# nextpyp/cet_pick

Measured on AMD Instinct MI355X. Metric: subtomograms/sec (MoCo-3D train) + voxels/sec (heatmap+NMS) at 1/2/4/8 GPU, higher is better.
Workload: dtype f32; 1 GPU; moco_main.py moco3d_18: 3D encoder, synthetic 512x512x128 tomogram, 32^3 subtomo crops, batch 64 per GPU, r=1024, dim=128, m=0.999, T=0.1, SGD lr 1e-3; global_batch=64, parallelism=dp1, hipgraph=True

## Files before the change

cet_pick_amd/_lib.py:

```python
import ctypes
import os

import torch

_HERE = os.path.dirname(os.path.abspath(__file__))
LIB_PATH = os.environ.get("CETPICK_HIP_LIB") or os.path.join(_HERE, "libcetpick_hip.so")

_c = ctypes
_P, _I, _F, _Z, _D, _L = _c.c_void_p, _c.c_int, _c.c_float, _c.c_size_t, _c.c_double, _c.c_long


class ConvGeom(ctypes.Structure):
    _fields_ = [(f, _I) for f in "N Di Hi Wi Ci Co kd kh kw stride pd ph pw dd dh dw".split()]


_G = _c.POINTER(ConvGeom)


class Aug2d3dRanges(ctypes.Structure):
    _fields_ = [(f, _F) for f in "flip_p angle_lo angle_hi erase_p scale_lo scale_hi ratio_lo ratio_hi".split()]


_R = _c.POINTER(Aug2d3dRanges)

# ... 127 lines not shown
    "mi_bn_bwd_apply": (_I, [_P, _P, _P, _P, _L, _I, _P, _P, _P, _D, _I, _P, _P, _P]),
    "mi_bn_bwd_apply_res": (_I, [_P, _P, _P, _P, _P, _L, _I, _P, _P, _P, _D, _P, _P, _P]),
    "mi_bn_param_grads": (_I, [_P, _I, _P, _P, _P]),
    "mi_colsum": (_I, [_P, _L, _I, _P, _P, _P, _Z, _P]),
    "mi_maxpool3d_fwd": (_I, [_P, _P, _P] + [_I] * 8 + [_P]),
    "mi_maxpool3d_bwd": (_I, [_P, _P, _P] + [_I] * 8 + [_P]),
    "mi_avgpool_fwd": (_I, [_P, _P, _I, _I, _I, _P]),
    "mi_avgpool_bwd": (_I, [_P, _P, _I, _I, _I, _P]),
    "mi_bias_add": (_I, [_P, _P, _L, _I, _P]),
    "mi_copy_pair_f32": (_I, [_P, _P, _P, _P, _L, _P]),
    "mi_relu_mask": (_I, [_P, _P, _P, _P, _L, _P]),
    "mi_l2norm_fwd": (_I, [_P, _P, _P, _I, _I, _P]),
    "mi_l2norm_bwd": (_I, [_P, _P, _P, _P, _I, _I, _P]),
    "mi_moco_logits_fwd": (_I, [_P, _P, _P, _P, _I, _I, _I, _F, _P]),
    "mi_moco_logits_norm_fwd": (_I, [_P, _P, _P, _P, _P, _P, _P, _I, _I, _I, _F, _P]),
    "mi_moco_logits_bwd": (_I, [_P, _P, _P, _P, _I, _I, _I, _F, _P]),
    "mi_rowdot_mean_fwd": (_I, [_P, _P, _P, _I, _I, _P]),
    "mi_rowdot_mean_bwd": (_I, [_P, _P, _P, _I, _I, _P]),
    "mi_column_std_mean": (_I, [_P, _P, _I, _I, _P]),
    "mi_ce_label0_fwd": (_I, [_P, _P, _P, _P, _P, _I, _I, _P, _P]),
    "mi_ce_label0_bwd": (_I, [_P, _P, _P, _P, _I, _I, _P]),
    "mi_conv3d_s2_dgrad_usable": (_I, [_I, _I, _I, _I]),
    "mi_conv3d_s2_dgrad_workspace_bytes": (_Z, [_I, _I]),
    "mi_conv3d_s2_dgrad_f32": (_I, [_P] * 7 + [_I, _I, _I, _I, _P, _Z, _P]),
    "mi_conv3d_s2_fwd_usable": (_I, [_I, _I, _I, _I]),
    "mi_conv3d_s2_fwd_workspace_bytes": (_Z, [_I, _I]),
    "mi_conv3d_s2_fwd_f32": (_I, [_P] * 5 + [_I, _I, _I, _I, _P, _Z, _P]),
    "mi_conv3d_s2_prep": (_I, [_P] * 6 + [_I, _P]),
    "mi_conv3d_s2_fwd_img_f32": (_I, [_P] * 4 + [_I] * 4 + [_P]),
    "mi_conv3d_s2_dgrad_img_f32": (_I, [_P] * 6 + [_I] * 4 + [_P]),
    "mi_ema_update": (_I, [_P, _P, _F, _L, _P]),
    "mi_sgd_step": (_I, [_P, _P, _P, _F, _F, _F, _L, _P]),
    "mi_sgd_step2": (_I, [_P, _P, _P, _P, _F, _F, _F, _L, _P]),
    "mi_scalar_accumulate": (_I, [_P, _P, _P, _P, _P, _P]),
    "mi_queue_enqueue": (_I, [_P, _P, _P, _I, _I, _I, _P]),
    "mi_kmeans_image_bytes": (_Z, [_I, _I]),
    "mi_kmeans_workspace_bytes": (_Z, [_L, _I, _I]),
    "mi_kmeans_prep": (_I, [_P, _I, _I, _P, _P]),
    "mi_kmeans_xnorm": (_I, [_P, _L, _I, _P, _P]),
    "mi_kmeans_assign": (_I, [_P, _P, _P, _L, _I, _I, _P, _P, _P, _Z, _P]),
    "mi_kmeans_update": (_I, [_P, _P, _L, _I, _I, _P, _P, _P, _P, _P, _Z, _P]),
    "mi_knn_image_bytes": (_Z, [_L, _I]),
    "mi_knn_workspace_bytes": (_Z, [_L, _L, _I, _I, _I, _I]),
    "mi_knn_search": (_I, [_P, _P, _L, _L, _I, _I, _I, _I, _I, _P, _P, _P, _Z, _P]),
    "mi_tsne_affinities": (_I, [_P, _L, _I, _F, _P, _P, _P]),
    "mi_tsne_workspace_bytes": (_Z, [_L, _I, _I]),
    "mi_tsne_gradient": (_I, [_P, _P, _P, _P, _P, _L, _I, _F, _I, _P, _P, _P, _P, _Z, _P]),
    "mi_tsne_update": (_I, [_P, _P, _P, _P, _L, _F, _F, _F, _P]),
    "mi_umap_check": (_I, [_L, _I]),
    "mi_umap_smooth_knn": (_I, [_P, _L, _I, _D, _P, _P, _P, _P]),
    "mi_umap_union": (_I, [_P, _P, _P, _P, _L, _I, _P, _I, _P, _P, _P, _P]),
    "mi_umap_rowmax": (_I, [_P, _P, _P, _P, _P, _L, _I, _D, _D, _P, _P]),
    "mi_umap_supervise": (_I, [_P, _P, _P, _P, _L, _I, _D, _D, _P, _I, _P, _P, _P]),
    "mi_umap_epoch": (_I, [_P, _P, _P, _P, _P, _P, _P, _L, _I, _I, _I, _D, _D, _c.c_uint64, _P]),
    "mi_graph_components": (_I, [_P, _P, _P, _P, _P, _L, _I, _P, _P, _P, _P]),
    "mi_spectral_degree": (_I, [_P, _P, _P, _P, _P, _P, _L, _I, _P, _P, _P]),
    "mi_spectral_spmv": (_I, [_P, _P, _P, _P, _P, _P, _L, _I, _P, _P, _P, _L, _L, _P]),
    "mi_spectral_workspace_bytes": (_Z, [_I, _L]),
    "mi_spectral_dots": (_I, [_P, _L, _I, _L, _P, _P, _P, _Z, _P]),
    "mi_spectral_orth": (_I, [_P, _L, _I, _L, _P, _P, _P, _Z, _P]),
    "mi_spectral_combine": (_I, [_P, _L, _I, _L, _P, _P, _D, _P]),
    "mi_vis_sample_colours": (_I, [_P, _L, _P, _I, _I, _P, _P]),
    "mi_vis_slice_bytes": (_I, [_P, _L, _L, _P, _D, _D, _P, _P]),
    "mi_vis_gauss_workspace_bytes": (_Z, [_L, _L, _L]),
    "mi_vis_gauss_u8": (_I, [_P, _I, _I, _I, _P, _P, _P, _Z, _P]),
    "mi_vis_paint": (_I, [_P, _P, _L, _P, _I, _I, _I, _I, _I, _I, _P, _P, _P]),
# ... 100 lines not shown
```

cet_pick_amd/csrc/conv_direct3.hip:

```cpp
#include "common.h"
#include "bf16x3.h"
#include <type_traits>
#include <algorithm>

namespace {

using namespace bf3;

constexpr int C = 64;
constexpr int PLANE = 64;
constexpr int TZ = 2;
constexpr int PZ = TZ + 2;
constexpr int NV = PZ * PLANE;
constexpr int LEAD = 16;
constexpr int ZREC = 34;
constexpr int NREC = LEAD + NV + ZREC;
constexpr int ARR = NREC * 16;
constexpr int KS = C / 16;
constexpr int PL_BYTES = 2 * ARR;
constexpr int KS_BYTES = 3 * PL_BYTES;
constexpr int LDS_BYTES = KS * KS_BYTES;
constexpr int ZBASE = (LEAD + NV) * 16;
constexpr int WBLK = 1024;
constexpr int WSTEP = 2 * 3 * WBLK;
constexpr int NTAP = 27;
constexpr int NSTEP = KS * NTAP;
constexpr int WIMG_BYTES = NSTEP * WSTEP;
constexpr int RB = 6;
static_assert(NSTEP % RB == 0, "ring slots");
static_assert(LDS_BYTES <= 160 * 1024, "patch must fit the CU's LDS");
static_assert(((LEAD + NV) & 15) == 0, "zero region must start at a record = 0 (mod 16)");

struct Direct3Params {
    const float* a;
// ... 399 lines not shown
            if (has_mask) v = (mm[r] > 0.f) ? v : 0.f;
            if (eo[r] != 0x80000000u) p.out[eo[r] / 4] = v;
        }
    }
}

constexpr int PREP_MAX = 16;
struct PrepBatch {
    const float* w[PREP_MAX];
    unsigned char* img[PREP_MAX];
    int dgrad[PREP_MAX];
    int wide[PREP_MAX];
};
__device__ void direct3s_prep_body(const float* w, unsigned char* img, int dgrad, int idx);
__device__ void direct3s256_prep_body(const float* w, unsigned char* img, int dgrad, int idx);
constexpr int PREP_BLOCKS_256 = 8 * NTAP * 2 * 8 * 64 / 256;
constexpr int PREP_BLOCKS = NTAP * KS * 2 * 64 / 256;
constexpr int PREP_BLOCKS_WIDE = 4 * NTAP * 2 * 4 * 64 / 256;
template <int CT>
__device__ void direct3_prep_body(const float* w, unsigned char* img, int dgrad, int idx) {
    constexpr int KSn = CT / 16;
    const int lane = idx & 63, cw = (idx >> 6) & 1, rest = idx >> 7, ks = rest % KSn, tap = (rest / KSn) % NTAP, cb = rest / (KSn * NTAP);
    if (cb >= CT / 64) return;
    const int nn = cb * 64 + cw * 32 + (lane & 31), k0 = ks * 16 + 8 * (lane >> 5);
    float v[8];
    if (dgrad) {
        ld8(w + ((long)(NTAP - 1 - tap) * CT + nn) * CT + k0, v);
    } else {
#pragma unroll
        for (int e = 0; e < 8; ++e) v[e] = w[((long)tap * CT + k0 + e) * CT + nn];
    }
    u32x4 o[3];
    cut8(v, o);
    unsigned char* dst = img + (long)(((cb * KSn + ks) * NTAP + tap) * 2 + cw) * (3 * WBLK) + lane * 16;
    store_planes(dst, WBLK, o);
}
__global__ __launch_bounds__(256) void direct3_prep_kernel(PrepBatch b) {
    const int fmt = b.wide[blockIdx.y], idx = blockIdx.x * 256 + threadIdx.x;
    if (fmt == 1) { if (blockIdx.x < PREP_BLOCKS_WIDE) direct3s_prep_body(b.w[blockIdx.y], b.img[blockIdx.y], b.dgrad[blockIdx.y], idx); }
    else if (fmt == 2) { if (blockIdx.x < PREP_BLOCKS_WIDE) direct3_prep_body<128>(b.w[blockIdx.y], b.img[blockIdx.y], b.dgrad[blockIdx.y], idx); }
    else if (fmt == 3) direct3s256_prep_body(b.w[blockIdx.y], b.img[blockIdx.y], b.dgrad[blockIdx.y], idx);
    else if (blockIdx.x < PREP_BLOCKS) direct3_prep_body<C>(b.w[blockIdx.y], b.img[blockIdx.y], b.dgrad[blockIdx.y], idx);
}

constexpr int WG_SPLITS = 28;
constexpr int WROW = 64;
constexpr int WHALF = (PLANE + 1) * WROW;
constexpr int WPL = 2 * WHALF;
constexpr int WOP = 3 * WPL;
constexpr int WBUF = 2 * WOP;
constexpr int WZERO = PLANE * WROW;

constexpr int WG_MAXPROB = 4;
struct Direct3WgradParams {
    const float* x[WG_MAXPROB];
    const float* dy[WG_MAXPROB];
    float* slabs[WG_MAXPROB];
    int N, D;
    unsigned bytes;
    int nprob, splits;
    int H, W;
};

constexpr int W_HB = 3 * 2 * 8 * 128;
template <bool V4, int CT, bool TILED = false>
__global__ __launch_bounds__(512, 2) void direct3_wgrad_kernel(Direct3WgradParams p) {
    __shared__ __attribute__((aligned(16))) unsigned char lds[2 * WBUF + (TILED ? 2 * W_HB : 16)];
    unsigned char* const halo = lds + 2 * WBUF;
// ... 423 lines not shown
    for (int i = 0; i < 2; ++i)
#pragma unroll
        for (int r = 0; r < 16; ++r) red[(cc * 32 + i * 16 + r) * 64 + lane] = acc[i][r];
    __syncthreads();
    const long m0 = (long)n0 * VS;
    const int col = ct * 32 + l32;
#pragma unroll
    for (int j = 0; j < 8; ++j) {
        const int idx = cc * 8 + j, i = idx >> 4, r = idx & 15;
        float t = ((red[idx * 64 + lane] + red[(32 + idx) * 64 + lane]) + red[(64 + idx) * 64 + lane]) + red[(96 + idx) * 64 + lane];
        const long o = (m0 + 32 * i + (r & 3) + 8 * (r >> 2) + 4 * h) * CT + col;
        if (p.res) t += p.res[o];
        if (p.relu) t = fmaxf(t, 0.f);
        if (p.mask) t = (p.mask[o] > 0.f) ? t : 0.f;
        p.out[o] = t;
    }
}

template <int CT>
__device__ void direct3s_prep_body_t(const float* w, unsigned char* img, int dgrad, int idx) {
    constexpr int NCB = CT / 32;
    const int lane = idx & 63, cb = (idx >> 6) % NCB, r1 = (idx >> 6) / NCB, ksx = r1 & 1, rest = r1 >> 1, tap = rest % NTAP, cc = rest / NTAP;
    if (cc >= NCB) return;
    const int nn = cb * 32 + (lane & 31), k0 = cc * 32 + ksx * 16 + 8 * (lane >> 5);
    float v[8];
    if (dgrad) {
        ld8(w + ((long)(NTAP - 1 - tap) * CT + nn) * CT + k0, v);
    } else {
#pragma unroll
        for (int e = 0; e < 8; ++e) v[e] = w[((long)tap * CT + k0 + e) * CT + nn];
    }
    u32x4 o[3];
    cut8(v, o);
    unsigned char* dst = img + (long)(((cc * NTAP + tap) * 2 + ksx) * NCB + cb) * (3 * WBLK) + lane * 16;
    store_planes(dst, WBLK, o);
}
__device__ void direct3s_prep_body(const float* w, unsigned char* img, int dgrad, int idx) { direct3s_prep_body_t<CS>(w, img, dgrad, idx); }
__device__ void direct3s256_prep_body(const float* w, unsigned char* img, int dgrad, int idx) { direct3s_prep_body_t<256>(w, img, dgrad, idx); }

}

int mi_direct3_kind(int N, int Di, int Hi, int Wi, int Ci, int Co, int kd, int kh, int kw, int stride, int pd, int ph,
                    int pw, int dd, int dh, int dw) {
    const char* off = getenv("MI_CONV_NO_DIRECT");
    if (off && atoi(off) != 0) return 0;
    if (kd != 3 || kh != 3 || kw != 3 || stride != 1 || pd != 1 || ph != 1 || pw != 1 || dd != 1 || dh != 1 || dw != 1) return 0;
    if (N < 1 || 4l * N * Di * Hi * Wi * Ci >= 0x7fff0000l) return 0;
    if (Ci == C && Co == C && Hi == 8 && Wi == 8 && Di >= TZ && Di % TZ == 0) return 1;
    if (Ci == CS && Co == CS && Di == 4 && Hi == 4 && Wi == 4) return 2;
    if (Ci == 128 && Co == 128 && Hi == 8 && Wi == 8 && Di >= TZ && Di % TZ == 0 && (long)N * Di >= 128 && (long)N * (Di / TZ) <= 0x7fffffffl) return 3;
    if (Ci == 256 && Co == 256 && Di == 4 && Hi == 4 && Wi == 4 && N >= 16) return 4;
    if (Ci == C && Co == C && (Hi > 8 || Wi > 8) && Hi >= 8 && Wi >= 8 && Di >= TZ && Di % TZ == 0) {
        const bool ragged = Hi % 8 != 0 || Wi % 8 != 0;
        const char* rg = getenv("MI_DIRECT3H_RAGGED");
        const long ty = (Hi + 7) / 8, tx = (Wi + 7) / 8, wgs = (long)N * (Di / TZ) * ty * tx;
        const bool fill_ok = 4l * Hi * Wi >= 3l * 64 * ty * tx;
        const bool take = !ragged || (rg ? atoi(rg) != 0 : fill_ok);
        if (wgs >= 128 && wgs <= 0x7fffffffl && take) return 5;
    }
    return 0;
}
bool mi_direct3_usable(int N, int Di, int Hi, int Wi, int Ci, int Co, int kd, int kh, int kw, int stride, int pd, int ph,
                       int pw, int dd, int dh, int dw) {
    return mi_direct3_kind(N, Di, Hi, Wi, Ci, Co, kd, kh, kw, stride, pd, ph, pw, dd, dh, dw) != 0;
}

size_t mi_direct3_wimg_bytes(int channels) {
    return channels == C ? (size_t)WIMG_BYTES : channels == CS ? (size_t)S_WIMG_BYTES : 0;
// ... 176 lines not shown
```

cet_pick_amd/csrc/train_ops.hip:

```cpp
#include "common.h"
#include "bf16x3.h"
#include <algorithm>

namespace {

using bf3::ld4;
using bf3::st4;

enum { CR_STATS = 0, CR_BNBWD = 1, CR_SUM = 2, CR_BNBWD_X = 3 };

struct PoolGeom { int N, Di, Hi, Wi, Do, Ho, Wo, k, s, pad; };

struct ColReduceParams {
    const float* a;
    const float* x;
    const float* y;
    const float* save;
    long M;
    int C, relu;
    double* partials;
    const float* gamma;
    const float* beta;
    double* sums_direct;
    float* f32_direct;
    int n_f32;
};

template <int MODE>
__global__ __launch_bounds__(256) void colreduce_kernel(ColReduceParams p) {
    const int CV = p.C >> 2;
    const int tcol = threadIdx.x % CV, trow = threadIdx.x / CV;
    const int RS = 256 / CV;
    float s0[4] = {0, 0, 0, 0}, s1[4] = {0, 0, 0, 0};
    double w0[4] = {0, 0, 0, 0}, w1[4] = {0, 0, 0, 0};
// ... 825 lines not shown
        row_lse[b] = m;
        row_lse[B + b] = ls;
        __hip_atomic_store(&row_loss[b], ce0_split(lse) ? (m - l[0]) + ls : lse - l[0], __ATOMIC_RELAXED,
                           __HIP_MEMORY_SCOPE_AGENT);
        __builtin_amdgcn_fence(__ATOMIC_RELEASE, "agent");
        asm volatile("s_waitcnt vmcnt(0)" ::: "memory");
        s_ticket = atomicAdd(counter ? counter : &g_ce0_arrivals, 1u);
    }
    __syncthreads();
    if (s_ticket == (unsigned)B - 1 && tid == 0) {
        __builtin_amdgcn_fence(__ATOMIC_ACQUIRE, "agent");
        float t = 0.f;
        for (int r = 0; r < B; ++r) t += __hip_atomic_load(&row_loss[r], __ATOMIC_RELAXED, __HIP_MEMORY_SCOPE_AGENT);
        *loss = t / (float)B;
        if (loss_copy) *loss_copy = t / (float)B;
        __hip_atomic_store(counter ? counter : &g_ce0_arrivals, 0u, __ATOMIC_RELAXED, __HIP_MEMORY_SCOPE_AGENT);
    }
}
__global__ __launch_bounds__(256) void ce0_bwd_kernel(const float* logits, const float* row_lse, const float* g_dev,
                                                     float* dlogits, int B, int n) {
    const int b = blockIdx.x;
    const float g = (*g_dev) / (float)B, m = row_lse[b], ls = row_lse[B + b], lse = m + ls;
    const bool split = ce0_split(lse);
    const float* l = logits + (long)b * n;
    for (int j = threadIdx.x; j < n; j += 256) {
        const float e = split ? expf((l[j] - m) - ls) : expf(l[j] - lse);
        dlogits[(long)b * n + j] = g * (e - (j == 0 ? 1.f : 0.f));
    }
}

__global__ __launch_bounds__(256) void ema_kernel(float* k, const float* q, float m, long n) {
    const float om = 1.0f - m;
    long n4 = n >> 2;
    for (long i = (long)blockIdx.x * 256 + threadIdx.x; i < n4; i += (long)gridDim.x * 256) {
        float4 a = ld4(k + 4 * i), b = ld4(q + 4 * i);
        a.x = a.x * m + b.x * om; a.y = a.y * m + b.y * om;
        a.z = a.z * m + b.z * om; a.w = a.w * m + b.w * om;
        st4(k + 4 * i, a);
    }
    if (blockIdx.x == 0)
        for (long i = (n4 << 2) + threadIdx.x; i < n; i += 256) k[i] = k[i] * m + q[i] * om;
}
__global__ __launch_bounds__(256) void sgd_kernel(float* p, const float* g, const float* lr_dev,
                                                 float lr_host, float wd, float gs, long n) {
    const float lr = lr_dev ? *lr_dev : lr_host;
    long n4 = n >> 2;
    for (long i = (long)blockIdx.x * 256 + threadIdx.x; i < n4; i += (long)gridDim.x * 256) {
        float4 a = ld4(p + 4 * i), b = ld4(g + 4 * i);
        a.x -= lr * (gs * b.x + wd * a.x); a.y -= lr * (gs * b.y + wd * a.y);
        a.z -= lr * (gs * b.z + wd * a.z); a.w -= lr * (gs * b.w + wd * a.w);
        st4(p + 4 * i, a);
    }
    if (blockIdx.x == 0)
        for (long i = (n4 << 2) + threadIdx.x; i < n; i += 256) p[i] -= lr * (gs * g[i] + wd * p[i]);
}

__global__ void enqueue_kernel(float* queue, long long* ptr, const float* keys, int B, int C, int R) {
    const long long p0 = *ptr;
    for (int i = blockIdx.x * blockDim.x + threadIdx.x; i < B * C; i += gridDim.x * blockDim.x) {
        int b = i % B, c = i / B;
        long long col = p0 + b;
        if (col < R) queue[(long)c * R + col] = keys[(long)b * C + c];
    }
}
__global__ void advance_ptr_kernel(long long* ptr, int B, int R) { *ptr = (*ptr + B) % R; }
__global__ __launch_bounds__(1024) void enqueue_small_kernel(float* queue, long long* ptr, const float* keys, int B, int C, int R) {
    const long long p0 = *ptr;
    for (int i = threadIdx.x; i < B * C; i += 1024) {
        int b = i % B, c = i / B;
        long long col = p0 + b;
        if (col < R) queue[(long)c * R + col] = keys[(long)b * C + c];
    }
    __syncthreads();
    if (threadIdx.x == 0) *ptr = (p0 + B) % R;
}

int ew_blocks(long n) { return (int)std::max<long>(1, std::min<long>((n + 255) / 256, 2048)); }

}

extern "C" size_t mi_colreduce_workspace_bytes(long M, int C) {
    if (!colreduce_ok(C)) return 0;
    return sizeof(double) * 2 * C * (size_t)colreduce_blocks(M, C);
}

extern "C" int mi_bn_stats(const float* x, long M, int C, double* sums, void* ws, size_t ws_bytes,
                           mi_stream_t stream) {
// ... 408 lines not shown

extern "C" int mi_ce_label0_fwd(const float* logits, float* loss, float* loss_copy, float* row_loss, float* row_lse, int B,
                                int n, unsigned* counter, mi_stream_t stream) {
    if (!logits || !loss || !row_loss || !row_lse || B <= 0 || n <= 0) return MI_E_ARG;
    hipLaunchKernelGGL(ce0_rows_kernel, dim3(B), dim3(256), 0, (hipStream_t)stream, logits, loss, loss_copy, row_loss, row_lse,
                       B, n, counter);
    MI_RETURN_IF_LAUNCH_FAILED();
    return MI_OK;
}
extern "C" int mi_ce_label0_bwd(const float* logits, const float* row_lse, const float* grad_loss, float* dlogits, int B,
                                int n, mi_stream_t stream) {
    if (!logits || !row_lse || !grad_loss || !dlogits || B <= 0 || n <= 0) return MI_E_ARG;
    hipLaunchKernelGGL(ce0_bwd_kernel, dim3(B), dim3(256), 0, (hipStream_t)stream, logits, row_lse, grad_loss, dlogits, B, n);
    MI_RETURN_IF_LAUNCH_FAILED();
    return MI_OK;
}

extern "C" int mi_ema_update(float* k, const float* q, float m, long n, mi_stream_t stream) {
    if (!k || !q || n <= 0 || ((uintptr_t)k & 15) || ((uintptr_t)q & 15)) return MI_E_ARG;
    hipLaunchKernelGGL(ema_kernel, dim3(ew_blocks(n / 4 + 1)), dim3(256), 0, (hipStream_t)stream, k, q, m, n);
    MI_RETURN_IF_LAUNCH_FAILED();
    return MI_OK;
}

extern "C" int mi_sgd_step(float* p, const float* g, const float* lr_dev, float lr, float weight_decay,
                           float grad_scale, long n, mi_stream_t stream) {
    if (!p || !g || n <= 0 || ((uintptr_t)p & 15) || ((uintptr_t)g & 15)) return MI_E_ARG;
    hipLaunchKernelGGL(sgd_kernel, dim3(ew_blocks(n / 4 + 1)), dim3(256), 0, (hipStream_t)stream, p, g, lr_dev, lr, weight_decay,
                       grad_scale, n);
    MI_RETURN_IF_LAUNCH_FAILED();
    return MI_OK;
}

__global__ __launch_bounds__(256) void sgd2_kernel(float* p, const float* g, const float* g2, const float* lr_dev, float lr_host, float wd,
                                                  float gs, long n) {
    const float lr = lr_dev ? *lr_dev : lr_host;
    long n4 = n >> 2;
    for (long i = (long)blockIdx.x * 256 + threadIdx.x; i < n4; i += (long)gridDim.x * 256) {
        float4 a = ld4(p + 4 * i), b = ld4(g + 4 * i), c = ld4(g2 + 4 * i);
        b.x += c.x; b.y += c.y; b.z += c.z; b.w += c.w;
        a.x -= lr * (gs * b.x + wd * a.x); a.y -= lr * (gs * b.y + wd * a.y);
        a.z -= lr * (gs * b.z + wd * a.z); a.w -= lr * (gs * b.w + wd * a.w);
        st4(p + 4 * i, a);
    }
    if (blockIdx.x == 0)
        for (long i = (n4 << 2) + threadIdx.x; i < n; i += 256) p[i] -= lr * (gs * (g[i] + g2[i]) + wd * p[i]);
}
extern "C" int mi_sgd_step2(float* p, const float* g, const float* g2, const float* lr_dev, float lr, float weight_decay,
                            float grad_scale, long n, mi_stream_t stream) {
    if (!p || !g || !g2 || n <= 0 || ((uintptr_t)p & 15) || ((uintptr_t)g & 15) || ((uintptr_t)g2 & 15)) return MI_E_ARG;
    hipLaunchKernelGGL(sgd2_kernel, dim3(ew_blocks(n / 4 + 1)), dim3(256), 0, (hipStream_t)stream, p, g, g2, lr_dev, lr, weight_decay,
                       grad_scale, n);
    MI_RETURN_IF_LAUNCH_FAILED();
    return MI_OK;
}

__global__ void scalar_accumulate_kernel(float* sums, const float* a, const float* b, const float* c, const float* d) {
    const float* src[4] = {a, b, c, d};
    const int i = threadIdx.x;
    if (i < 4 && src[i]) sums[i] += *src[i];
}
extern "C" int mi_scalar_accumulate(float* sums, const float* a, const float* b, const float* c, const float* d, mi_stream_t stream) {
    if (!sums) return MI_E_ARG;
    hipLaunchKernelGGL(scalar_accumulate_kernel, dim3(1), dim3(64), 0, (hipStream_t)stream, sums, a, b, c, d);
    MI_RETURN_IF_LAUNCH_FAILED();
    return MI_OK;
// ... 18 lines not shown
```

cet_pick_amd/hipops.py:

```python
import collections
import ctypes
import math
import os
import torch
import torch.nn as nn

from . import _lib as L


PROFILE = None
PROFILE_REPEAT = 8


def _prof_run(tag, flops, fn):
    fn()
    if PROFILE is not None:
        e0 = torch.cuda.Event(enable_timing=True)
        e1 = torch.cuda.Event(enable_timing=True)
        e0.record()
        for _ in range(PROFILE_REPEAT):
            fn()
        e1.record()
        PROFILE.append((tag, flops, e0, e1, PROFILE_REPEAT))

# ... 225 lines not shown
        return _ws(L.lib().mi_conv_workspace_bytes(self.ref), device, "conv")


def _linear_geom(m, ci, co):
    return _Geom((m, 1, 1, 1, ci), co, (1, 1, 1), 1, (0, 0, 0))


ACTIVE_IMAGES = None

_ImageFamily = collections.namedtuple("_ImageFamily", ("nbytes", "prep"))
_IMAGE_FAMILIES = {
    "s2": _ImageFamily(lambda lib, w, dgrad: (lib.mi_conv3d_s2_dgrad_workspace_bytes if dgrad else lib.mi_conv3d_s2_fwd_workspace_bytes)(
        int(w.shape[1]), int(w.shape[0])), "mi_conv3d_s2_prep"),
    "direct": _ImageFamily(lambda lib, w, dgrad: lib.mi_conv3d_direct_wimg_bytes(int(w.shape[0])), "mi_conv3d_direct_prep"),
    "p2d": _ImageFamily(lambda lib, w, dgrad: lib.mi_conv2d_p2d_wimg_bytes(int(w.shape[0])), "mi_conv2d_p2d_prep"),
}


def _prep_images(family, items):
    if not items:
        return
    fn = _IMAGE_FAMILIES[family].prep
    ints = lambda vals: L.host_array(vals, ctypes.c_int)
    w, img = L.host_array([it[0].data_ptr() for it in items]), L.host_array([it[3].data_ptr() for it in items])
    dgrad, co = ints([it[2] for it in items]), ints([int(it[0].shape[0]) for it in items])
    if family == "s2":
        args = (w, L.host_array([(it[1].data_ptr() if it[1] is not None else None) for it in items]), img,
                ints([int(it[0].shape[1]) for it in items]), co, dgrad)
    else:
        args = (w, img, dgrad, co)
    L.check(getattr(L.lib(), fn)(*args, len(items), L.stream()), fn)


class WeightImages:
    def __init__(self):
        self._groups = {}
        self._by_weight = {}

    @staticmethod
    def eligible(w, k, stride, pad):
        return (w.is_cuda and tuple(w.shape[:2]) in ((64, 64), (128, 128)) and _k3(k, True) == (3, 3, 3) and stride == 1
                and _p3(pad, True) == (1, 1, 1) and _phys_ok(w))

    def add(self, group, family, w, dgrad, w_ds=None):
        dgrad = int(bool(dgrad))
        img = torch.empty(int(_IMAGE_FAMILIES[family].nbytes(L.lib(), w, dgrad)), dtype=torch.uint8, device=w.device)
        self._groups.setdefault(group, {f: [] for f in _IMAGE_FAMILIES})[family].append((w, w_ds, dgrad, img))
        self._by_weight[(family, w.data_ptr(), dgrad)] = img

    def get(self, family, w, dgrad):
        return self._by_weight.get((family, w.data_ptr(), int(bool(dgrad))))

    def refresh(self, group):
        for family, items in self._groups.get(group, {}).items():
            _prep_images(family, items)

    def refresh_all(self):
        for group in self._groups:
            self.refresh(group)

    def versions(self):
        return sum(it[0]._version + (it[1]._version if it[1] is not None else 0)
                   for g in self._groups.values() for items in g.values() for it in items)


def _held_image(w, dgrad):
    if ACTIVE_IMAGES is not None:
        for family in _IMAGE_FAMILIES:
            img = ACTIVE_IMAGES.get(family, w, dgrad)
            if img is not None:
                return family, img
    return None, None


def _switch(name):
    value = os.environ.get(name, "")
    return value.startswith("f") if name == "MI_CONV_ARITH" else bool(value)


def _arith_bf16x3():
    return not _switch("MI_CONV_ARITH")


SMALLK = os.environ.get("CETPICK_SMALLK", "1") != "0"

WEIGHT_EPOCH = 0


def _bump_weight_epoch():
    global WEIGHT_EPOCH
    WEIGHT_EPOCH += 1

# ... 1503 lines not shown
    return _CELabel0Fn.apply(_f32c(logits, "logits"), out)


class _RowDotMeanFn(torch.autograd.Function):

    @staticmethod
    def forward(ctx, a, b):
        bsz, c = a.shape
        out = torch.empty((), dtype=torch.float32, device=a.device)
        L.check(L.lib().mi_rowdot_mean_fwd(L.ptr(a), L.ptr(b), L.ptr(out), bsz, c, L.stream()), "mi_rowdot_mean_fwd")
        ctx.save_for_backward(b)
        return out

    @staticmethod
    def backward(ctx, g):
        (b,) = ctx.saved_tensors
        da = torch.empty_like(b)
        L.check(L.lib().mi_rowdot_mean_bwd(L.ptr(b), L.ptr(g.contiguous()), L.ptr(da), b.shape[0], b.shape[1],
                                           L.stream()), "mi_rowdot_mean_bwd")
        return da, None


def rowdot_mean(a, b):
    return _RowDotMeanFn.apply(_f32c(a, "a"), _f32c(b, "b"))


def column_std_mean(x):
    out = torch.empty((), dtype=torch.float32, device=x.device)
    L.check(L.lib().mi_column_std_mean(L.ptr(_f32c(x, "x")), L.ptr(out), x.shape[0], x.shape[1], L.stream()),
            "mi_column_std_mean")
    return out


def ema_update_(k_flat, q_flat, m):
    _bump_weight_epoch()
    L.check(L.lib().mi_ema_update(L.ptr(k_flat), L.ptr(q_flat), float(m), k_flat.numel(), L.stream()),
            "mi_ema_update")


def sgd_step_(p_flat, g_flat, lr, weight_decay=0.0, lr_dev=None, grad_scale=1.0):
    _bump_weight_epoch()
    L.check(L.lib().mi_sgd_step(L.ptr(p_flat), L.ptr(g_flat), L.ptr(lr_dev), float(lr), float(weight_decay),
                                float(grad_scale), p_flat.numel(), L.stream()), "mi_sgd_step")


def sgd_step2_(p_flat, g_flat, g2_flat, lr, weight_decay=0.0, lr_dev=None, grad_scale=1.0):
    _bump_weight_epoch()
    L.check(L.lib().mi_sgd_step2(L.ptr(p_flat), L.ptr(g_flat), L.ptr(g2_flat), L.ptr(lr_dev), float(lr), float(weight_decay),
                                 float(grad_scale), p_flat.numel(), L.stream()), "mi_sgd_step2")


def scalar_accumulate_(sums, *scalars):
    if len(scalars) > 4 or sums.numel() < len(scalars):
        raise L.HipExtensionError("scalar_accumulate_: at most four scalars, sums at least as long")
    ptrs = [L.ptr(_f32c(t, "scalar")) for t in scalars] + [None] * (4 - len(scalars))
    L.check(L.lib().mi_scalar_accumulate(L.ptr(sums), *ptrs, L.stream()), "mi_scalar_accumulate")


def copy_pair_(dst0, src0, dst1, src1):
    ts = (dst0, src0, dst1, src1)
    if (all(t.is_cuda and t.dtype == torch.float32 and t.is_contiguous() for t in ts) and src0.shape == dst0.shape
            and src1.shape == dst1.shape and dst0.numel() == dst1.numel() and dst0.numel() % 4 == 0
            and all(t.data_ptr() % 16 == 0 for t in ts)):
        L.check(L.lib().mi_copy_pair_f32(L.ptr(dst0), L.ptr(src0), L.ptr(dst1), L.ptr(src1), dst0.numel(), L.stream()),
                "mi_copy_pair_f32")
        return
    dst0.copy_(src0)
    dst1.copy_(src1)


def queue_enqueue_(queue, queue_ptr, keys):
    c, r = queue.shape
    b = keys.shape[0]
    if r % b != 0:
# ... 517 lines not shown
```

cet_pick_amd/models/moco.py:

```python
import torch
import torch.nn as nn

from .. import hipops as H


class MoCo(nn.Module):
    def __init__(self, encoder_q, encoder_k, dim=32, r=1024, m=0.999, T=0.1):
        super().__init__()
        self.r, self.m, self.T = r, m, T
        self.encoder_q = encoder_q
        self.encoder_k = encoder_k
        for param_q, param_k in zip(self.encoder_q.parameters(), self.encoder_k.parameters()):
            param_k.data.copy_(param_q.data)
            param_k.requires_grad = False
        self.register_buffer("queue", torch.randn(dim, r))
        self.queue = nn.functional.normalize(self.queue, dim=0)
        self.register_buffer("queue_ptr", torch.zeros(1, dtype=torch.long))
        self._arena_q = self._arena_k = None

    def flatten_parameters(self):
        if self._arena_q is None or self._arena_q.flat.device != next(self.encoder_q.parameters()).device:
            self._arena_q = H.ParamArena(self.encoder_q)
            self._arena_k = H.ParamArena(self.encoder_k)
            assert self._arena_q.numel == self._arena_k.numel
        return self._arena_q, self._arena_k

    @torch.no_grad()
    def _momentum_update_key_encoder(self):
        if self._arena_q is not None:
            H.ema_update_(self._arena_k.flat, self._arena_q.flat, self.m)
            if self.weight_images is not None and H.ACTIVE_IMAGES is self.weight_images:
                self.weight_images.refresh("k")
            return
        for param_q, param_k in zip(self.encoder_q.parameters(), self.encoder_k.parameters()):
            n = param_q.numel()
            q = torch.as_strided(param_q.data, (n,), (1,))
            k = torch.as_strided(param_k.data, (n,), (1,))
            if n % 4 == 0 and k.data_ptr() % 16 == 0 and q.data_ptr() % 16 == 0:
                H.ema_update_(k, q, self.m)
            else:
                k.mul_(self.m).add_(q, alpha=1.0 - self.m)

    @torch.no_grad()
    def _dequeue_and_enqueue(self, keys):
        H.queue_enqueue_(self.queue, self.queue_ptr, keys.contiguous())

    overlap_key_branch = True
    _side = None
    weight_images = None

    def _zero_labels(self, logits):
        lab = getattr(self, "_labels", None)
        if lab is None or lab.shape[0] != logits.shape[0] or lab.device != logits.device:
            lab = torch.zeros(logits.shape[0], dtype=torch.long, device=logits.device)
            self._labels = lab
        return lab

    def _key_branch(self, im_k):
        with torch.no_grad():
            self._momentum_update_key_encoder()
            H.stamp("ema")
            k = self.encoder_k(im_k)[0]["proj"]
            return k

# ... 147 lines not shown
```

cet_pick_amd/trains/moco_engine.py:

```python
import os

import torch

from .. import hipops as H
from .step_graph import StepGraph


class MocoStepEngine(StepGraph):
    def __init__(self, moco, lr, weight_decay=0.0, use_graph=False):
        self.moco = moco
        self.arena_q, self.arena_k = moco.flatten_parameters()
        super().__init__(moco, [self.arena_q, self.arena_k], lr, weight_decay, use_graph)
        dev = self.arena_q.flat.device
        self.logits = None
        self._one = torch.ones((), dtype=torch.float32, device=dev)
        self.loss = torch.zeros((), dtype=torch.float32, device=dev)
        self._loss_buf = self.loss
        self.loss_sum = torch.zeros((), dtype=torch.float32, device=dev)
        self._xchg = None
        self.buckets_sent = []
        if self.dist_on:
            self._setup_buckets()
        self.side_wgrads = dev.type == "cuda" and os.environ.get("CETPICK_SIDE_WGRADS", "1") != "0"
        self._wside = None
# ... 96 lines not shown
        moco = self.moco
        self.buckets_sent = []
        self.arena_q.zero_grad()
        H.ACTIVE_IMAGES = self._images
        moco.defer_enqueue = True
        try:
            H.stamp("step:start")
            logits, labels = moco(im_q, im_k)
            self.logits = logits.detach()
            loss = H.cross_entropy_label0(logits, out=self._loss_buf)
            H.DEFERRED_WGRADS = [] if self.arena_q.flat_grad.is_cuda else None
            H.SIDE_WGRADS = [] if self.side_wgrads else None
            self._wside_used = False
            loss.backward(self._one)
            if H.SIDE_WGRADS:
                H.run_wgrad_jobs(H.SIDE_WGRADS)
            H.SIDE_WGRADS = None
            if self._wside_used:
                torch.cuda.current_stream().wait_stream(self._wside)
            del self._wside_keep[:]
            H.stamp("backward:end")
            H.flush_wgrad_reduces()
            moco.flush_enqueue()
        finally:
            H.DEFERRED_WGRADS = None
            H.SIDE_WGRADS = None
            H.ACTIVE_IMAGES = None
            moco.defer_enqueue = False
            moco._pending_keys = None
        if self.dist_on:
            self._reduce_bucket("stem")
            if self._xchg is not None:
                torch.cuda.current_stream().wait_stream(self._xchg)
        H.sgd_step_(self.arena_q.flat, self.arena_q.flat_grad, self.lr, self.weight_decay, self.lr_dev,
                    grad_scale=1.0 / self.world)
        if self._images is not None:
            self._images.refresh("q")
        self.loss_sum.add_(self.loss)
        H.stamp("step:end")
        return self.loss

    def take_loss_sum(self):
        v = float(self.loss_sum.item())
        self.loss_sum.zero_()
        return v
```

include/cetpick_hip.h:

```cpp
#ifndef CETPICK_HIP_H
#define CETPICK_HIP_H

#include <stddef.h>
#include <stdint.h>

#ifdef __cplusplus
extern "C" {
#endif

typedef void* mi_stream_t;

#define MI_OK 0
#define MI_E_ARG (-1)
#define MI_E_WORKSPACE (-2)
#define MI_E_UNSUPPORTED (-3)

int mi_abi_version(void);
int mi_graph_node_counts(void* graph, int* counts);
int mi_debug_stamp(void* slot, mi_stream_t stream);
const char* mi_debug_last_conv_kernel(void);
int mi_debug_last_conv_plan(int* out, int n);
const char* mi_build_arch(void);


// ... 259 lines not shown
                       int C, int R, float T, mi_stream_t stream);
int mi_moco_logits_norm_fwd(const float* q_raw, const float* k_raw, const float* queue, float* logits, float* q_hat,
                            float* q_inv, float* k_hat, int B, int C, int R, float T, mi_stream_t stream);
int mi_moco_logits_bwd(const float* dlogits, const float* k, const float* queue, float* dq, int B,
                       int C, int R, float T, mi_stream_t stream);
int mi_rowdot_mean_fwd(const float* a, const float* b, float* out, int B, int C, mi_stream_t stream);
int mi_rowdot_mean_bwd(const float* b, const float* grad_out, float* da, int B, int C, mi_stream_t stream);
int mi_column_std_mean(const float* x, float* out, int B, int C, mi_stream_t stream);
int mi_ce_label0_fwd(const float* logits, float* loss, float* loss_copy ,
                     float* row_loss, float* row_lse, int B, int n, unsigned* counter, mi_stream_t stream);
int mi_ce_label0_bwd(const float* logits, const float* row_lse, const float* grad_loss, float* dlogits, int B, int n,
                     mi_stream_t stream);

int mi_conv3d_s2_dgrad_usable(int N, int Gi, int Ci, int Co);
size_t mi_conv3d_s2_dgrad_workspace_bytes(int Ci, int Co);
int mi_conv3d_s2_dgrad_f32(const float* dh, const float* dout, const float* w, const float* w_ds, float* dx, const float* res,
                           const float* mask, int N, int Gi, int Ci, int Co, void* ws, size_t ws_bytes, mi_stream_t stream);

int mi_conv3d_s2_fwd_usable(int N, int Gi, int Ci, int Co);
size_t mi_conv3d_s2_fwd_workspace_bytes(int Ci, int Co);
int mi_conv3d_s2_fwd_f32(const float* x, const float* w, const float* w_ds, float* hmid, float* r, int N, int Gi, int Ci, int Co,
                         void* ws, size_t ws_bytes, mi_stream_t stream);

int mi_conv3d_s2_prep(const float* const* w, const float* const* w_ds, void* const* img, const int* ci, const int* co,
                      const int* dgrad, int n, mi_stream_t stream);
int mi_conv3d_s2_fwd_img_f32(const float* x, const void* img, float* hmid, float* r, int N, int Gi, int Ci, int Co,
                             mi_stream_t stream);
int mi_conv3d_s2_dgrad_img_f32(const float* dh, const float* dout, const void* img, float* dx, const float* res,
                               const float* mask, int N, int Gi, int Ci, int Co, mi_stream_t stream);

int mi_ema_update(float* k, const float* q, float m, long n, mi_stream_t stream);
int mi_sgd_step(float* p, const float* g, const float* lr_dev, float lr, float weight_decay, float grad_scale, long n,
                mi_stream_t stream);
int mi_sgd_step2(float* p, const float* g, const float* g2, const float* lr_dev, float lr, float weight_decay, float grad_scale, long n,
                 mi_stream_t stream);
int mi_scalar_accumulate(float* sums, const float* a, const float* b, const float* c, const float* d, mi_stream_t stream);
int mi_queue_enqueue(float* queue, int64_t* queue_ptr, const float* keys, int B, int C, int R,
                     mi_stream_t stream);

size_t mi_voxel_loss_workspace_bytes(long n);
int mi_pu_focal_loss_fwd(const float* pred, const float* gt, long n, double tau, double beta, double* sums,
                         float* loss, void* ws, size_t ws_bytes, mi_stream_t stream);
int mi_pu_focal_loss_bwd(const float* pred, const float* gt, long n, double tau, const double* sums,
                         const float* dloss, float* dpred, mi_stream_t stream);
int mi_focal_loss_fwd(const float* pred, const float* gt, long n, double* sums, float* loss, void* ws,
                      size_t ws_bytes, mi_stream_t stream);
int mi_focal_loss_bwd(const float* pred, const float* gt, long n, const double* sums, const float* dloss,
                      float* dpred, mi_stream_t stream);
int mi_mse_loss_fwd(const float* a, const float* b, long n, double* sums, float* loss, void* ws,
                    size_t ws_bytes, mi_stream_t stream);
int mi_mse_loss_bwd(const float* a, const float* b, long n, const double* sums, const float* dloss, float* da,
                    float* db, mi_stream_t stream);
int mi_ucl_rowsums_fwd(const float* feat, const uint8_t* cls, int n2, int dim, float inv_T, float* rowmax,
                       float* s_all, float* s_pos, float* s_other, float* e_pair, mi_stream_t stream);
int mi_ucl_rowsums_bwd_ranged(const float* feat, const uint8_t* cls, int n2, int dim, float inv_T, const float* rowmax,
                              const float* g_all, const float* g_pos, const float* g_other, const float* g_pair, float* dfeat,
                              float* range, mi_stream_t stream);

size_t mi_kmeans_image_bytes(int d, int k);
size_t mi_kmeans_workspace_bytes(long n, int d, int k);
int mi_kmeans_prep(const float* centroids, int d, int k, void* image, mi_stream_t stream);
int mi_kmeans_xnorm(const float* x, long n, int d, float* xnorm, mi_stream_t stream);
int mi_kmeans_assign(const float* x, const float* xnorm, const void* image, long n, int d, int k, int32_t* labels,
                     float* dist, void* ws, size_t ws_bytes, mi_stream_t stream);
int mi_kmeans_update(const float* x, const int32_t* labels, long n, int d, int k, float* centroids, int32_t* counts,
                     float* obj, int32_t* nsplit, void* ws, size_t ws_bytes, mi_stream_t stream);
// ... 77 lines not shown
```

Baseline: 41980 subtomograms/sec.

## Fuse optimizer step and EMA with conv weight-image regeneration in one kernel

```diff
diff --git a/cet_pick_amd/_lib.py b/cet_pick_amd/_lib.py
--- a/cet_pick_amd/_lib.py
+++ b/cet_pick_amd/_lib.py
@@ -183,6 +183,8 @@
     "mi_ema_update": (_I, [_P, _P, _F, _L, _P]),
     "mi_sgd_step": (_I, [_P, _P, _P, _F, _F, _F, _L, _P]),
     "mi_sgd_step2": (_I, [_P, _P, _P, _P, _F, _F, _F, _L, _P]),
+    "mi_sgd_step_images": (_I, [_P, _P, _P, _F, _F, _F, _L, _P, _I, _L, _I, _P, _P, _P]),
+    "mi_ema_update_images": (_I, [_P, _P, _F, _L, _P, _I, _L, _I, _P]),
     "mi_scalar_accumulate": (_I, [_P, _P, _P, _P, _P, _P]),
     "mi_queue_enqueue": (_I, [_P, _P, _P, _I, _I, _I, _P]),
     "mi_kmeans_image_bytes": (_Z, [_I, _I]),
diff --git a/cet_pick_amd/csrc/conv_direct3.hip b/cet_pick_amd/csrc/conv_direct3.hip
--- a/cet_pick_amd/csrc/conv_direct3.hip
+++ b/cet_pick_amd/csrc/conv_direct3.hip
@@ -1,5 +1,6 @@
 #include "common.h"
 #include "bf16x3.h"
+#include "weight_image.h"
 #include <type_traits>
 #include <algorithm>
 
@@ -465,8 +466,7 @@
     }
     u32x4 o[3];
     cut8(v, o);
-    unsigned char* dst = img + (long)(((cb * KSn + ks) * NTAP + tap) * 2 + cw) * (3 * WBLK) + lane * 16;
-    store_planes(dst, WBLK, o);
+    store_planes(img + wimg::direct3_entry<CT>(tap, k0, nn), WBLK, o);
 }
 __global__ __launch_bounds__(256) void direct3_prep_kernel(PrepBatch b) {
     const int fmt = b.wide[blockIdx.y], idx = blockIdx.x * 256 + threadIdx.x;
@@ -956,8 +956,7 @@
     }
     u32x4 o[3];
     cut8(v, o);
-    unsigned char* dst = img + (long)(((cc * NTAP + tap) * 2 + ksx) * NCB + cb) * (3 * WBLK) + lane * 16;
-    store_planes(dst, WBLK, o);
+    store_planes(img + wimg::direct3s_entry<CT>(tap, k0, nn), WBLK, o);
 }
 __device__ void direct3s_prep_body(const float* w, unsigned char* img, int dgrad, int idx) { direct3s_prep_body_t<CS>(w, img, dgrad, idx); }
 __device__ void direct3s256_prep_body(const float* w, unsigned char* img, int dgrad, int idx) { direct3s_prep_body_t<256>(w, img, dgrad, idx); }
diff --git a/cet_pick_amd/csrc/optim_update.h b/cet_pick_amd/csrc/optim_update.h
--- /dev/null
+++ b/cet_pick_amd/csrc/optim_update.h
@@ -0,0 +1,22 @@
+#pragma once
+#include <hip/hip_runtime.h>
+
+namespace optim {
+
+__device__ __forceinline__ float sgd1(float p, float g, float lr, float wd, float gs) {
+    p -= lr * (gs * g + wd * p);
+    return p;
+}
+__device__ __forceinline__ float4 sgd4(float4 a, const float4 b, float lr, float wd, float gs) {
+    a.x -= lr * (gs * b.x + wd * a.x); a.y -= lr * (gs * b.y + wd * a.y);
+    a.z -= lr * (gs * b.z + wd * a.z); a.w -= lr * (gs * b.w + wd * a.w);
+    return a;
+}
+__device__ __forceinline__ float ema1(float k, float q, float m, float om) { return k * m + q * om; }
+__device__ __forceinline__ float4 ema4(float4 a, const float4 b, float m, float om) {
+    a.x = a.x * m + b.x * om; a.y = a.y * m + b.y * om;
+    a.z = a.z * m + b.z * om; a.w = a.w * m + b.w * om;
+    return a;
+}
+
+}
diff --git a/cet_pick_amd/csrc/train_ops.hip b/cet_pick_amd/csrc/train_ops.hip
--- a/cet_pick_amd/csrc/train_ops.hip
+++ b/cet_pick_amd/csrc/train_ops.hip
@@ -1,5 +1,7 @@
 #include "common.h"
 #include "bf16x3.h"
+#include "optim_update.h"
+#include "weight_image.h"
 #include <algorithm>
 
 namespace {
@@ -891,27 +893,105 @@
 __global__ __launch_bounds__(256) void ema_kernel(float* k, const float* q, float m, long n) {
     const float om = 1.0f - m;
     long n4 = n >> 2;
-    for (long i = (long)blockIdx.x * 256 + threadIdx.x; i < n4; i += (long)gridDim.x * 256) {
-        float4 a = ld4(k + 4 * i), b = ld4(q + 4 * i);
-        a.x = a.x * m + b.x * om; a.y = a.y * m + b.y * om;
-        a.z = a.z * m + b.z * om; a.w = a.w * m + b.w * om;
-        st4(k + 4 * i, a);
-    }
+    for (long i = (long)blockIdx.x * 256 + threadIdx.x; i < n4; i += (long)gridDim.x * 256)
+        st4(k + 4 * i, optim::ema4(ld4(k + 4 * i), ld4(q + 4 * i), m, om));
     if (blockIdx.x == 0)
-        for (long i = (n4 << 2) + threadIdx.x; i < n; i += 256) k[i] = k[i] * m + q[i] * om;
+        for (long i = (n4 << 2) + threadIdx.x; i < n; i += 256) k[i] = optim::ema1(k[i], q[i], m, om);
 }
 __global__ __launch_bounds__(256) void sgd_kernel(float* p, const float* g, const float* lr_dev,
                                                  float lr_host, float wd, float gs, long n) {
     const float lr = lr_dev ? *lr_dev : lr_host;
     long n4 = n >> 2;
-    for (long i = (long)blockIdx.x * 256 + threadIdx.x; i < n4; i += (long)gridDim.x * 256) {
-        float4 a = ld4(p + 4 * i), b = ld4(g + 4 * i);
-        a.x -= lr * (gs * b.x + wd * a.x); a.y -= lr * (gs * b.y + wd * a.y);
-        a.z -= lr * (gs * b.z + wd * a.z); a.w -= lr * (gs * b.w + wd * a.w);
-        st4(p + 4 * i, a);
-    }
+    for (long i = (long)blockIdx.x * 256 + threadIdx.x; i < n4; i += (long)gridDim.x * 256)
+        st4(p + 4 * i, optim::sgd4(ld4(p + 4 * i), ld4(g + 4 * i), lr, wd, gs));
     if (blockIdx.x == 0)
-        for (long i = (n4 << 2) + threadIdx.x; i < n; i += 256) p[i] -= lr * (gs * g[i] + wd * p[i]);
+        for (long i = (n4 << 2) + threadIdx.x; i < n; i += 256) p[i] = optim::sgd1(p[i], g[i], lr, wd, gs);
+}
+
+constexpr int BOUNDARY_MAX_SEGS = 64;
+constexpr int TROW = 68;
+struct BoundaryParams {
+    float* a;
+    const float* b;
+    const float* lr_dev;
+    float lr_host, wd, gs, m;
+    long n;
+    const long long* plan;
+    float* loss_sum;
+    const float* loss;
+    int tiles;
+};
+template <bool SGD>
+__global__ __launch_bounds__(256) void step_boundary_kernel(BoundaryParams p) {
+    __shared__ __attribute__((aligned(16))) float T[64 * TROW];
+    __shared__ long long seg[2 * (BOUNDARY_MAX_SEGS + 1)];
+    const int tid = threadIdx.x;
+    const float lr = SGD ? (p.lr_dev ? *p.lr_dev : p.lr_host) : 0.f, om = 1.0f - p.m;
+    const int nw = (int)p.plan[0];
+    if ((int)blockIdx.x >= p.tiles) {
+        const int ns = (int)p.plan[1];
+        const long total = p.plan[3];
+        for (int i = tid; i < 2 * (ns + 1); i += 256) seg[i] = p.plan[4 + 5 * nw + i];
+        __syncthreads();
+        const long ab = blockIdx.x - p.tiles, nab = gridDim.x - p.tiles;
+        int s = 0;
+        long shift = seg[0] - seg[1], next = seg[3];
+        for (long j = ab * 256 + tid; j < total; j += nab * 256) {
+            if (j >= next) {
+                while (seg[2 * (s + 1) + 1] <= j) ++s;
+                shift = seg[2 * s] - seg[2 * s + 1]; next = seg[2 * (s + 1) + 1];
+            }
+            const long i = j + shift;
+            float* ap = p.a + 4 * i;
+            const float4 a = ld4(ap), b = ld4(p.b + 4 * i);
+            st4(ap, SGD ? optim::sgd4(a, b, lr, p.wd, p.gs) : optim::ema4(a, b, p.m, om));
+        }
+        if (ab == 0) {
+            for (long i = ((p.n >> 2) << 2) + tid; i < p.n; i += 256)
+                p.a[i] = SGD ? optim::sgd1(p.a[i], p.b[i], lr, p.wd, p.gs) : optim::ema1(p.a[i], p.b[i], p.m, om);
+            if (SGD && p.loss_sum && tid == 0) *p.loss_sum += *p.loss;
+        }
+        return;
+    }
+    int wi = 0;
+    while (wi + 1 < nw && (int)p.plan[4 + 5 * (wi + 1) + 2] <= (int)blockIdx.x) ++wi;
+    const long long* w = p.plan + 4 + 5 * wi;
+    const int ch = (int)w[1], t = (int)blockIdx.x - (int)w[2];
+    unsigned char* fwd = reinterpret_cast<unsigned char*>(w[3]);
+    unsigned char* dgr = reinterpret_cast<unsigned char*>(w[4]);
+    const bool wide = ch == 128;
+    const int tap = wide ? t >> 2 : t, ci0 = wide ? ((t >> 1) & 1) * 64 : 0, co0 = wide ? (t & 1) * 64 : 0;
+    const long t0 = w[0] + ((long)tap * ch + ci0) * ch + co0;
+#pragma unroll
+    for (int i = 0; i < 4; ++i) {
+        const int f = tid + 256 * i, r = f >> 4, c = (f & 15) * 4;
+        const long o = t0 + (long)r * ch + c;
+        const float4 a = ld4(p.a + o), b = ld4(p.b + o);
+        const float4 v = SGD ? optim::sgd4(a, b, lr, p.wd, p.gs) : optim::ema4(a, b, p.m, om);
+        st4(p.a + o, v);
+        *reinterpret_cast<float4*>(&T[r * TROW + c]) = v;
+    }
+    __syncthreads();
+#pragma unroll
+    for (int i = 0; i < 2; ++i) {
+        const int ent = tid + 256 * i, x = ent & 63, g8 = (ent >> 6) * 8;
+        float v[8];
+        bf3::u32x4 o[3];
+        if (fwd) {
+#pragma unroll
+            for (int e = 0; e < 8; ++e) v[e] = T[(g8 + e) * TROW + x];
+            bf3::cut8(v, o);
+            bf3::store_planes(fwd + (wide ? wimg::direct3s_entry<128>(tap, ci0 + g8, co0 + x) : wimg::direct3_entry<64>(tap, ci0 + g8, co0 + x)),
+                              wimg::WBLK, o);
+        }
+        if (dgr) {
+            bf3::ld8(&T[x * TROW + g8], v);
+            bf3::cut8(v, o);
+            const int dt = wimg::NTAP - 1 - tap;
+            bf3::store_planes(dgr + (wide ? wimg::direct3s_entry<128>(dt, co0 + g8, ci0 + x) : wimg::direct3_entry<64>(dt, co0 + g8, ci0 + x)),
+                              wimg::WBLK, o);
+        }
+    }
 }
 
 __global__ void enqueue_kernel(float* queue, long long* ptr, const float* keys, int B, int C, int R) {
@@ -1386,6 +1466,28 @@
     return MI_OK;
 }
 
+static int step_boundary_launch(bool sgd, BoundaryParams p, long unowned4, int n_segs, hipStream_t s) {
+    if (!p.a || !p.b || !p.plan || p.n <= 0 || ((uintptr_t)p.a & 15) || ((uintptr_t)p.b & 15)) return MI_E_ARG;
+    if (p.tiles < 0 || unowned4 < 0 || unowned4 > (p.n >> 2) || n_segs < 0 || n_segs > BOUNDARY_MAX_SEGS) return MI_E_ARG;
+    if ((p.loss_sum == nullptr) != (p.loss == nullptr)) return MI_E_ARG;
+    const dim3 grid((unsigned)(p.tiles + ew_blocks(unowned4 + 1)));
+    if (sgd) hipLaunchKernelGGL(step_boundary_kernel<true>, grid, dim3(256), 0, s, p);
+    else hipLaunchKernelGGL(step_boundary_kernel<false>, grid, dim3(256), 0, s, p);
+    MI_RETURN_IF_LAUNCH_FAILED();
+    return MI_OK;
+}
+extern "C" int mi_sgd_step_images(float* p, const float* g, const float* lr_dev, float lr, float weight_decay, float grad_scale, long n,
+                                  const int64_t* plan, int tiles, long unowned4, int n_segs, float* loss_sum, const float* loss,
+                                  mi_stream_t stream) {
+    BoundaryParams bp = {p, g, lr_dev, lr, weight_decay, grad_scale, 0.f, n, (const long long*)plan, loss_sum, loss, tiles};
+    return step_boundary_launch(true, bp, unowned4, n_segs, (hipStream_t)stream);
+}
+extern "C" int mi_ema_update_images(float* k, const float* q, float m, long n, const int64_t* plan, int tiles, long unowned4, int n_segs,
+                                    mi_stream_t stream) {
+    BoundaryParams bp = {k, q, nullptr, 0.f, 0.f, 0.f, m, n, (const long long*)plan, nullptr, nullptr, tiles};
+    return step_boundary_launch(false, bp, unowned4, n_segs, (hipStream_t)stream);
+}
+
 __global__ __launch_bounds__(256) void sgd2_kernel(float* p, const float* g, const float* g2, const float* lr_dev, float lr_host, float wd,
                                                   float gs, long n) {
     const float lr = lr_dev ? *lr_dev : lr_host;
diff --git a/cet_pick_amd/csrc/weight_image.h b/cet_pick_amd/csrc/weight_image.h
--- /dev/null
+++ b/cet_pick_amd/csrc/weight_image.h
@@ -0,0 +1,20 @@
+#pragma once
+#include <hip/hip_runtime.h>
+
+namespace wimg {
+
+constexpr int NTAP = 27;
+constexpr int WBLK = 1024;
+
+template <int CT>
+__device__ __forceinline__ long direct3_entry(int tap, int k0, int nn) {
+    const int cb = nn >> 6, cw = (nn >> 5) & 1, ks = k0 >> 4, lane = (nn & 31) | (((k0 >> 3) & 1) << 5);
+    return (long)(((cb * (CT / 16) + ks) * NTAP + tap) * 2 + cw) * (3 * WBLK) + lane * 16;
+}
+template <int CT>
+__device__ __forceinline__ long direct3s_entry(int tap, int k0, int nn) {
+    const int cb = nn >> 5, cc = k0 >> 5, ksx = (k0 >> 4) & 1, lane = (nn & 31) | (((k0 >> 3) & 1) << 5);
+    return (long)(((cc * NTAP + tap) * 2 + ksx) * (CT / 32) + cb) * (3 * WBLK) + lane * 16;
+}
+
+}
diff --git a/cet_pick_amd/hipops.py b/cet_pick_amd/hipops.py
--- a/cet_pick_amd/hipops.py
+++ b/cet_pick_amd/hipops.py
@@ -281,10 +281,18 @@
     L.check(getattr(L.lib(), fn)(*args, len(items), L.stream()), fn)
 
 
+_BoundaryPlan = collections.namedtuple("_BoundaryPlan", ("table", "tiles", "unowned4", "n_segs", "rest"))
+
+
+def fused_boundary():
+    return PROFILE is None and os.environ.get("CETPICK_FUSED_BOUNDARY", "1") != "0"
+
+
 class WeightImages:
     def __init__(self):
         self._groups = {}
         self._by_weight = {}
+        self._plans = {}
 
     @staticmethod
     def eligible(w, k, stride, pad):
@@ -296,6 +304,7 @@
         img = torch.empty(int(_IMAGE_FAMILIES[family].nbytes(L.lib(), w, dgrad)), dtype=torch.uint8, device=w.device)
         self._groups.setdefault(group, {f: [] for f in _IMAGE_FAMILIES})[family].append((w, w_ds, dgrad, img))
         self._by_weight[(family, w.data_ptr(), dgrad)] = img
+        self._plans.clear()
 
     def get(self, family, w, dgrad):
         return self._by_weight.get((family, w.data_ptr(), int(bool(dgrad))))
@@ -307,6 +316,49 @@
     def refresh_all(self):
         for group in self._groups:
             self.refresh(group)
+
+    def boundary_plan(self, group, flat):
+        key = (group, flat.data_ptr(), flat.numel())
+        plan = self._plans.get(key)
+        if plan is not None:
+            return plan
+        n, base = flat.numel(), flat.data_ptr()
+        owned, rest = {}, {}
+        for family, items in self._groups.get(group, {}).items():
+            for it in items:
+                w, dgrad, img = it[0], it[2], it[3]
+                off, ch = (w.data_ptr() - base) // 4, int(w.shape[0])
+                inside = (family == "direct" and w.dtype == torch.float32 and (w.data_ptr() - base) % 16 == 0 and ch in (64, 128)
+                          and 0 <= off and off + 27 * ch * ch <= n)
+                if inside:
+                    owned.setdefault(off, [ch, 0, 0])[1 + dgrad] = img.data_ptr()
+                else:
+                    rest.setdefault(family, []).append(it)
+        offs = sorted(owned)
+        for a, b in zip(offs, offs[1:]):
+            if a + 27 * owned[a][0] ** 2 > b:
+                raise L.HipExtensionError("cached weights overlap in the arena")
+        if len(offs) + 1 > 64:
+            raise L.HipExtensionError("more than 63 cached weights in one arena")
+        table, segs, tiles, cur4, un4 = [], [], 0, 0, 0
+        for off in offs:
+            ch, fwd, dg = owned[off]
+            table += [off, ch, tiles, fwd, dg]
+            tiles += 27 * (ch // 64) ** 2
+            segs += [cur4, un4]
+            un4 += off // 4 - cur4
+            cur4 = (off + 27 * ch * ch) // 4
+        segs += [cur4, un4]
+        un4 += n // 4 - cur4
+        segs += [n // 4, un4]
+        dev = torch.tensor([len(offs), len(offs) + 1, tiles, un4] + table + segs, dtype=torch.int64, device=flat.device)
+        plan = _BoundaryPlan(dev, tiles, un4, len(offs) + 1, rest)
+        self._plans[key] = plan
+        return plan
+
+    def refresh_rest(self, plan):
+        for family, items in plan.rest.items():
+            _prep_images(family, items)
 
     def versions(self):
         return sum(it[0]._version + (it[1]._version if it[1] is not None else 0)
@@ -1876,14 +1928,27 @@
     return out
 
 
-def ema_update_(k_flat, q_flat, m):
+def ema_update_(k_flat, q_flat, m, images=None, group=None):
     _bump_weight_epoch()
+    if images is not None and k_flat.is_cuda:
+        plan = images.boundary_plan(group, k_flat)
+        L.check(L.lib().mi_ema_update_images(L.ptr(k_flat), L.ptr(q_flat), float(m), k_flat.numel(), L.ptr(plan.table), plan.tiles,
+                                             plan.unowned4, plan.n_segs, L.stream()), "mi_ema_update_images")
+        images.refresh_rest(plan)
+        return
     L.check(L.lib().mi_ema_update(L.ptr(k_flat), L.ptr(q_flat), float(m), k_flat.numel(), L.stream()),
             "mi_ema_update")
 
 
-def sgd_step_(p_flat, g_flat, lr, weight_decay=0.0, lr_dev=None, grad_scale=1.0):
+def sgd_step_(p_flat, g_flat, lr, weight_decay=0.0, lr_dev=None, grad_scale=1.0, images=None, group=None, loss_sum=None, loss=None):
     _bump_weight_epoch()
+    if images is not None and p_flat.is_cuda:
+        plan = images.boundary_plan(group, p_flat)
+        L.check(L.lib().mi_sgd_step_images(L.ptr(p_flat), L.ptr(g_flat), L.ptr(lr_dev), float(lr), float(weight_decay), float(grad_scale),
+                                           p_flat.numel(), L.ptr(plan.table), plan.tiles, plan.unowned4, plan.n_segs,
+                                           L.ptr(loss_sum), L.ptr(loss), L.stream()), "mi_sgd_step_images")
+        images.refresh_rest(plan)
+        return
     L.check(L.lib().mi_sgd_step(L.ptr(p_flat), L.ptr(g_flat), L.ptr(lr_dev), float(lr), float(weight_decay),
                                 float(grad_scale), p_flat.numel(), L.stream()), "mi_sgd_step")
 
diff --git a/cet_pick_amd/models/moco.py b/cet_pick_amd/models/moco.py
--- a/cet_pick_amd/models/moco.py
+++ b/cet_pick_amd/models/moco.py
@@ -28,8 +28,12 @@
     @torch.no_grad()
     def _momentum_update_key_encoder(self):
         if self._arena_q is not None:
+            in_step = self.weight_images is not None and H.ACTIVE_IMAGES is self.weight_images
+            if in_step and H.fused_boundary():
+                H.ema_update_(self._arena_k.flat, self._arena_q.flat, self.m, images=self.weight_images, group="k")
+                return
             H.ema_update_(self._arena_k.flat, self._arena_q.flat, self.m)
-            if self.weight_images is not None and H.ACTIVE_IMAGES is self.weight_images:
+            if in_step:
                 self.weight_images.refresh("k")
             return
         for param_q, param_k in zip(self.encoder_q.parameters(), self.encoder_k.parameters()):
diff --git a/cet_pick_amd/trains/moco_engine.py b/cet_pick_amd/trains/moco_engine.py
--- a/cet_pick_amd/trains/moco_engine.py
+++ b/cet_pick_amd/trains/moco_engine.py
@@ -152,11 +152,15 @@
             self._reduce_bucket("stem")
             if self._xchg is not None:
                 torch.cuda.current_stream().wait_stream(self._xchg)
-        H.sgd_step_(self.arena_q.flat, self.arena_q.flat_grad, self.lr, self.weight_decay, self.lr_dev,
-                    grad_scale=1.0 / self.world)
-        if self._images is not None:
-            self._images.refresh("q")
-        self.loss_sum.add_(self.loss)
+        if self._images is not None and H.fused_boundary():
+            H.sgd_step_(self.arena_q.flat, self.arena_q.flat_grad, self.lr, self.weight_decay, self.lr_dev,
+                        grad_scale=1.0 / self.world, images=self._images, group="q", loss_sum=self.loss_sum, loss=self.loss)
+        else:
+            H.sgd_step_(self.arena_q.flat, self.arena_q.flat_grad, self.lr, self.weight_decay, self.lr_dev,
+                        grad_scale=1.0 / self.world)
+            if self._images is not None:
+                self._images.refresh("q")
+            self.loss_sum.add_(self.loss)
         H.stamp("step:end")
         return self.loss
 
diff --git a/include/cetpick_hip.h b/include/cetpick_hip.h
--- a/include/cetpick_hip.h
+++ b/include/cetpick_hip.h
@@ -315,6 +315,11 @@
 int mi_ema_update(float* k, const float* q, float m, long n, mi_stream_t stream);
 int mi_sgd_step(float* p, const float* g, const float* lr_dev, float lr, float weight_decay, float grad_scale, long n,
                 mi_stream_t stream);
+int mi_sgd_step_images(float* p, const float* g, const float* lr_dev, float lr, float weight_decay, float grad_scale, long n,
+                       const int64_t* plan, int tiles, long unowned4, int n_segs, float* loss_sum, const float* loss,
+                       mi_stream_t stream);
+int mi_ema_update_images(float* k, const float* q, float m, long n, const int64_t* plan, int tiles, long unowned4, int n_segs,
+                         mi_stream_t stream);
 int mi_sgd_step2(float* p, const float* g, const float* g2, const float* lr_dev, float lr, float weight_decay, float grad_scale, long n,
                  mi_stream_t stream);
 int mi_scalar_accumulate(float* sums, const float* a, const float* b, const float* c, const float* d, mi_stream_t stream);
```

After: 42150 subtomograms/sec, median of 6. Within noise of the previous version (+0.4%).
